# pdh930105/ARCQuant

Hardware: AMD Instinct MI355X
Metric: ARC-NVFP4 GEMM TFLOP/s (M=4096, N=KQ=4096, KE=64) (higher is better)
Workload: dtype f16

## Files before the change

arcquant_amd/agemm.py:

```python
from __future__ import annotations

import functools

import torch

from . import _lib
from ._lib import VARIANT_G16, VARIANT_G32, OUT_BF16, OUT_F32, ArcqError

_raw_stream = getattr(torch._C, "_cuda_getCurrentRawStream", None)


def _stream(t: torch.Tensor) -> int:
    if _raw_stream is not None:
        return _raw_stream(t.get_device())
    return torch.cuda.current_stream(t.device).cuda_stream


class _on:
    __slots__ = ("ctx",)

    def __init__(self, device):
        idx = device.index
        self.ctx = None if idx is None or idx == torch.cuda.current_device() else torch.cuda.device(device)

# ... 50 lines not shown

_OUT_CODES = {torch.bfloat16: OUT_BF16, torch.float32: OUT_F32}


def _out(out, M, N, out_dtype, like, who):
    code = _OUT_CODES.get(out_dtype)
    if code is None:
        raise RuntimeError(f"agemm.{who}: out_dtype must be bfloat16 or float32")
    if out is None:
        return torch.empty((M, N), dtype=out_dtype, device=like.device), code
    _need(out, out_dtype, "out", 2)
    if out.shape != (M, N):
        raise RuntimeError(f"agemm.{who}: out has the wrong shape, expected ({M}, {N})")
    return out, code


def _same_device(who: str, A: torch.Tensor, *ts):
    idx = A.get_device()
    if idx < 0:
        raise RuntimeError(f"agemm.{who}: the operands must live on the GPU (there is no CPU path)")
    for t in ts:
        if t is not None and t.get_device() != idx:
            raise RuntimeError(f"agemm.{who}: every operand must live on the GPU of the first one ({A.device}), got {t.device}")


@functools.lru_cache(maxsize=None)
def variant_for_kq(KQ: int) -> int:
    return int(_lib.lib().arcq_variant_for_kq(int(KQ)))


@functools.lru_cache(maxsize=None)
def sf_buffer_bytes(rows: int, K: int) -> int:
    return int(_lib.lib().arcq_sf_alloc_bytes(int(rows), int(K)))


@functools.lru_cache(maxsize=None)
def _sf_used(rows: int, K: int) -> int:
    return int(_lib.lib().arcq_sf_used_bytes(int(rows), int(K)))


@functools.lru_cache(maxsize=None)
def _repacked_bytes(N: int, K: int):
    L = _lib.lib()
    return int(L.arcq_repacked_w_bytes(N, K)), int(L.arcq_repacked_sf_bytes(N, K))


# ... 485 lines not shown
```

arcquant_amd/csrc/arcq_internal.hpp:

```cpp
#pragma once
#include <hip/hip_runtime.h>
#include <stdint.h>
#include <stdlib.h>

#include "../../include/arcq.h"

namespace arcq {

int fail(int code, const char* fmt, ...) __attribute__((format(printf, 2, 3)));

inline int env_int(const char* name, int dflt) {
  const char* e = getenv(name);
  return e ? atoi(e) : dflt;
}

constexpr int kMaxDevices = 64;
struct LdsOptIn {
  int granted[kMaxDevices];
};
int ensure_dynamic_lds(const void* kernel, LdsOptIn& cache, int bytes, const char* who);

struct LdsBytes {
  int launch, optin;
  LdsBytes(int bytes) : launch(bytes), optin(bytes) {}
// ... 99 lines not shown
  const uint8_t* RSF;
  void* D;
  uint32_t* out_slots;
  const int16_t* act_scatter;
  int M, N, KQ, KE, variant;
  float alpha_host;
  const float* alpha_dev;
  const uint16_t* bias;
  const uint16_t* residual;
  int out_dtype;
};
int gemm_fused_supported(int kind, int64_t M, int64_t N, int64_t KQ, int64_t KE);
int gemm_fused(const FusedArgs& f, hipStream_t stream);
int64_t gemm_skinny_workspace_bytes(int64_t M, int64_t N, int64_t K);
int64_t gemm_tile_workspace_bytes(int64_t M, int64_t N, int64_t K);
int64_t gemm_tile_silu_slots(int64_t M, int64_t N, int64_t K);
int64_t gemm_decode_silu_slots(int64_t M, int64_t N, int64_t K);
int gemm_splitk_finish(const GemmArgs& a, int splitk, hipStream_t stream);
int gemm_skinny(const GemmArgs& a, hipStream_t stream);
int64_t gemm_decode_workspace_bytes(int64_t M, int64_t N, int64_t K);
int gemm_decode(const GemmArgs& a, hipStream_t stream);
int gemm_tile(const GemmArgs& a, hipStream_t stream);
int gemm_tile_repacked(const GemmArgs& a, hipStream_t stream);
int gemm_regtile_cfg(int64_t M, int64_t N, int64_t K, int epilogue);
int gemm_regtile(const GemmArgs& a, int cfg, hipStream_t stream);
int gemm_regtile_fits(int64_t M, int64_t N, int64_t K, int b_layout);

struct KvWriteArgs {
  void* kv_data;
  void* kv_param;
  const int32_t *kv_indptr, *kv_indices, *last_page_offset;
  const void *k, *v, *k_param, *v_param;
  const int32_t* seqlen_indptr;
  int64_t ntok, B, L, layer, N, P;
  int format, dtype;
  bool quantize;
};
int kv_write(const KvWriteArgs& a, hipStream_t stream);
struct KvDecodeArgs {
  void* o;
  const void *q, *kv_data, *kv_param;
  const int32_t *kv_indptr, *kv_indices, *last_page_offset;
  int64_t B, Nq, L, layer, N, P, nnz;
  int format, dtype;
  void* workspace;
};
// ... 23 lines not shown
```

arcquant_amd/csrc/c_api.hip:

```cpp
#include <hip/hip_runtime.h>
#include <stdarg.h>
#include <stdio.h>
#include <string.h>

#include "arcq_device.hpp"
#include "arcq_internal.hpp"

namespace arcq {

static thread_local char g_err[512] = "";

int fail(int code, const char* fmt, ...) {
  va_list ap;
  va_start(ap, fmt);
  vsnprintf(g_err, sizeof(g_err), fmt, ap);
  va_end(ap);
  return code;
}

int ensure_dynamic_lds(const void* kernel, LdsOptIn& cache, int bytes, const char* who) {
  if (bytes <= 48 * 1024) return ARCQ_OK;
  int dev = 0;
  if (hipGetDevice(&dev) != hipSuccess) return fail(ARCQ_ERR_LAUNCH, "%s: hipGetDevice failed", who);
  const bool cached = dev >= 0 && dev < kMaxDevices;
// ... 95 lines not shown
                        int64_t M, int64_t KQ, int64_t KE, int variant, void* stream) {
  return quantize_x_dyn(X, reorder_index, QX, SFX, scale_out, state, M, KQ, KE, variant, (hipStream_t)stream);
}

int arcq_silu_mul_quantize_x_dyn(const void* GU, const int16_t* reorder_index, uint8_t* QX, uint8_t* SFX, float* scale_out, void* state,
                                 int64_t M, int64_t KQ, int64_t KE, int variant, int layout, void* stream) {
  return silu_mul_quantize_x_dyn(GU, reorder_index, QX, SFX, scale_out, state, M, KQ, KE, variant, layout, (hipStream_t)stream);
}

int arcq_absmax_scale(const void* X, int64_t n, float* scale_out, void* stream) {
  return absmax_scale(X, n, scale_out, (hipStream_t)stream);
}


static bool use_decode_v2(int64_t N) {
  static const int forced = env_int("ARCQ_DECODE", 0);
  if (forced == 1) return false;
  if (forced == 2) return true;
  return ((N + 127) / 128) * 4 >= 160;
}

int64_t arcq_gemm_workspace_bytes(int64_t M, int64_t N, int64_t K) {
  if (M <= 0 || N <= 0 || K <= 0) return 0;
  if (gemm_regtile_cfg(M, N, K, kEpiPlain)) return 0;
  if (M <= kSkinnyMaxM) return use_decode_v2(N) ? gemm_decode_workspace_bytes(M, N, K) : gemm_skinny_workspace_bytes(M, N, K);
  return gemm_tile_workspace_bytes(M, N, K);
}

int arcq_gemm_nvfp4(const uint8_t* A, const uint8_t* B, const uint8_t* SFA, const uint8_t* SFB, void* D, int64_t M, int64_t N,
                    int64_t K, float alpha_host, const float* alpha_dev, const void* bias, const void* residual, int out_dtype, void* workspace,
                    int64_t workspace_bytes, void* stream) {
  GemmRule r{"arcq_gemm_nvfp4"};
  const int rc = gemm_checks(r, A, B, SFA, SFB, D, nullptr, M, N, K, bias, residual, out_dtype);
  if (rc != ARCQ_OK) return rc < 0 ? rc : ARCQ_OK;
  const GemmArgs a = gemm_args(A, B, SFA, SFB, D, M, N, K, alpha_host, alpha_dev, bias, residual, out_dtype, workspace, workspace_bytes);
  if (const int cfg = gemm_regtile_cfg(M, N, K, kEpiPlain)) return gemm_regtile(a, cfg, (hipStream_t)stream);
  if (M <= kSkinnyMaxM) return use_decode_v2(N) ? gemm_decode(a, (hipStream_t)stream) : gemm_skinny(a, (hipStream_t)stream);
  return gemm_tile(a, (hipStream_t)stream);
}

int64_t arcq_gemm_silu_mul_slots(int64_t M, int64_t N, int64_t K) {
  if (M <= 0 || N <= 0 || K <= 0) return 0;
  return M <= kSkinnyMaxM ? gemm_decode_silu_slots(M, N, K) : gemm_tile_silu_slots(M, N, K);
}

int arcq_gemm_nvfp4_silu_mul(const uint8_t* A, const uint8_t* B, const uint8_t* SFA, const uint8_t* SFB, void* ACT, uint32_t* absmax_slots,
                             int64_t M, int64_t N, int64_t K, float alpha_host, const float* alpha_dev, const void* bias, void* stream) {
  GemmRule r{"arcq_gemm_nvfp4_silu_mul"};
  r.n_mult = 8; r.d = "ACT"; r.slots = true;
  const int rc = gemm_checks(r, A, B, SFA, SFB, ACT, absmax_slots, M, N, K, nullptr, nullptr, ARCQ_OUT_BF16);
  if (rc != ARCQ_OK) return rc < 0 ? rc : ARCQ_OK;
  GemmArgs a = gemm_args(A, B, SFA, SFB, ACT, M, N, K, alpha_host, alpha_dev, bias, nullptr, ARCQ_OUT_BF16, nullptr, 0);
  a.epilogue = kEpiSiluMul; a.absmax_slots = absmax_slots;
  if (bias && M <= kSkinnyMaxM) return fail(ARCQ_ERR_UNSUPPORTED, "%s: bias is supported by the tile kernel only (M > 16); decode uses arcq_linear_rmsnorm_silu_repacked", r.who);
  if (M <= kSkinnyMaxM) return gemm_decode(a, (hipStream_t)stream);
  return gemm_tile(a, (hipStream_t)stream);
}

// ... 25 lines not shown
int arcq_gemm_nvfp4_repacked_stream(const uint8_t* A, const uint8_t* RW, const uint8_t* SFA, const uint8_t* RSF, void* D, int64_t M, int64_t N,
                                    int64_t K, float alpha_host, const float* alpha_dev, const void* bias, const void* residual, int out_dtype,
                                    void* stream) {
  return gemm_repacked_entry(true, "arcq_gemm_nvfp4_repacked_stream", A, RW, SFA, RSF, D, M, N, K, alpha_host, alpha_dev, bias, residual, out_dtype, stream);
}

int arcq_gemm_nvfp4_repacked_silu_absmax(const uint8_t* A, const uint8_t* RW, const uint8_t* SFA, const uint8_t* RSF, void* D,
                                         uint32_t* absmax_slots, int64_t M, int64_t N, int64_t K, float alpha_host, const float* alpha_dev,
                                         void* stream) {
  GemmRule r{"arcq_gemm_nvfp4_repacked_silu_absmax"};
  r.n_mult = 4; r.max_m = 0; r.b = "RW"; r.sfb = "RSF"; r.slots = true;
  const int rc = gemm_checks(r, A, RW, SFA, RSF, D, absmax_slots, M, N, K, nullptr, nullptr, ARCQ_OUT_BF16);
  if (rc != ARCQ_OK) return rc < 0 ? rc : ARCQ_OK;
  GemmArgs a = gemm_args(A, nullptr, SFA, nullptr, D, M, N, K, alpha_host, alpha_dev, nullptr, nullptr, ARCQ_OUT_BF16, nullptr, 0);
  a.epilogue = kEpiSiluMul; a.absmax_slots = absmax_slots;
  return gemm_repacked(a, RW, RSF, (hipStream_t)stream);
}

static const int kRwDecodeCfg = 9;

static int rw_route(int64_t M, int64_t N, int64_t K, bool epi_aligned, int* cfg) {
  *cfg = 0;
  if (M <= 0 || N <= 0 || K <= 0 || (K % 64) || M > INT32_MAX / 2 || N > INT32_MAX / 2 || K > INT32_MAX / 2 || M * N > ((int64_t)1 << 40)) return 0;
  if (epi_aligned && gemm_repacked_supported(M, N, K)) return 1;
  *cfg = gemm_regtile_cfg(M, N, K, kEpiPlain);
  if (*cfg == 0 && M <= kSkinnyMaxM) *cfg = kRwDecodeCfg;
  if (*cfg) return gemm_regtile_fits(M, N, K, kBRepacked) ? 2 : 0;
  return 3;
}

int arcq_gemm_rw_route(int64_t M, int64_t N, int64_t K) {
  int cfg;
  return rw_route(M, N, K, true, &cfg);
}

int64_t arcq_gemm_rw_workspace_bytes(int64_t M, int64_t N, int64_t K) {
  int cfg;
  return rw_route(M, N, K, false, &cfg) == 3 ? gemm_tile_workspace_bytes(M, N, K) : 0;
}

int arcq_gemm_nvfp4_rw(const uint8_t* A, const uint8_t* RW, const uint8_t* SFA, const uint8_t* RSF, void* D, int64_t M, int64_t N, int64_t K,
                       float alpha_host, const float* alpha_dev, const void* bias, const void* residual, int out_dtype, void* workspace,
                       int64_t workspace_bytes, void* stream) {
  GemmRule r{"arcq_gemm_nvfp4_rw"};
  r.b = "RW"; r.sfb = "RSF";
  const int rc = gemm_checks(r, A, RW, SFA, RSF, D, nullptr, M, N, K, nullptr, nullptr, out_dtype);
// ... 108 lines not shown
```

arcquant_amd/csrc/gemm_tile.hip:

```cpp
#include <hip/hip_runtime.h>
#include <stdint.h>
#include <stdlib.h>

#include <type_traits>

#include "arcq_internal.hpp"
#include "gemm_common.hpp"
#include "gemm_tile_common.hpp"

namespace arcq {

#ifdef ARCQ_STREAM_STAMPS
static unsigned long long* g_tile_stamps = nullptr;
#ifndef ARCQ_TILE_REPACKED_UNIT
extern "C" void arcq_debug_set_tile_stamps(void* p) { g_tile_stamps = reinterpret_cast<unsigned long long*>(p); }
#endif
#define ARCQ_TILE_STAMP(k)                                                                                     \
  do {                                                                                                         \
    if (p.stamps && tid == 0) {                                                                                \
      unsigned long long t0_, t1_;                                                                             \
      asm volatile("s_memtime %0\n\ts_memrealtime %1\n\ts_waitcnt lgkmcnt(0)" : "=s"(t0_), "=s"(t1_)::"memory"); \
      p.stamps[(size_t)blockIdx.x * (2 * kTileStamps) + 2 * (k)] = t0_;                                        \
      p.stamps[(size_t)blockIdx.x * (2 * kTileStamps) + 2 * (k) + 1] = t1_;                                    \
    }                                                                                                          \
  } while (0)
#else
#define ARCQ_TILE_STAMP(k) do { } while (0)
#endif

#ifndef ARCQ_TILE_WIDE_STORES
#define ARCQ_TILE_WIDE_STORES 1
#endif

#ifndef ARCQ_TILE_BARRIER_AT_STEP_END
#define ARCQ_TILE_BARRIER_AT_STEP_END 0
#endif
#ifndef ARCQ_TILE_ROT
#define ARCQ_TILE_ROT 1
#endif

template <int BM, int BN, int WAVES_M, int WAVES_N, bool kMfma32, int kEpi, bool kStagger, bool kPipe, int kBLayout = kBRef>
__global__ __launch_bounds__(WAVES_M* WAVES_N * 64) void gemm_tile_kernel(TileParams p) {
  constexpr int kThreads = WAVES_M * WAVES_N * 64;
  constexpr int WM = BM / WAVES_M, WN = BN / WAVES_N;
  constexpr int kT = kMfma32 ? 32 : 16;
  constexpr int TM = WM / kT, TN = WN / kT;
  using acc_t = typename std::conditional<kMfma32, f32x16, f32x4>::type;
  constexpr int A_UNITS = (BM * 2 + kThreads - 1) / kThreads, B_UNITS = (BN * 2 + kThreads - 1) / kThreads;
  constexpr bool A_PARTIAL = (BM * 2) % kThreads != 0, B_PARTIAL = (BN * 2) % kThreads != 0;
  static_assert(!A_PARTIAL || A_UNITS == 1, "a partial A pass is a single pass");
  static_assert(!B_PARTIAL || B_UNITS == 1, "a partial B pass is a single pass");
  constexpr int A_TILE = BM * kRowBytes, B_TILE = BN * kRowBytes;

  extern __shared__ __attribute__((aligned(16))) unsigned char smem[];
  unsigned char* const lds_a0 = smem;
  unsigned char* const lds_b0 = smem + A_TILE;
  unsigned char* const lds_a1 = smem + A_TILE + B_TILE;
  unsigned char* const lds_b1 = smem + 2 * A_TILE + B_TILE;

  const int ntiles = p.tiles_m * p.tiles_n;
  int bid = blockIdx.x, split = 0;
  if (p.splits > 1) {
    split = bid / ntiles;
    bid -= split * ntiles;
  }
// ... 50 lines not shown
  }
  uint32_t b_q[B_UNITS], b_sf[B_UNITS];
  uint32_t b_live[B_UNITS];
  int b_slot[B_UNITS][4];
#pragma unroll
  for (int u = 0; u < B_UNITS; ++u) {
    const int unit = tid + u * kThreads, r = B_PARTIAL ? min(unit >> 1, BN - 1) : unit >> 1, h = unit & 1;
    const int row = n0 + r, rc = row < p.N ? row : p.N - 1;
    if constexpr (kBLayout == kBRepacked) {
      const uint32_t rb = (uint32_t)((rc >> 4) - (n0 >> 4));
      b_q[u] = rb * (uint32_t)rw_tiles * 1024u + h * 256 + (rc & 15) * 16;
      b_sf[u] = rb * (uint32_t)rw_tiles * 128u + h * 64 + (rc & 15) * 4;
    } else {
      b_q[u] = (uint32_t)(rc - n0) * (uint32_t)half_k + h * 16;
      b_sf[u] = (uint32_t)(sf_atom_offset(rc, 0, atoms_k) - sf_atom_offset(n0, 0, atoms_k)) + h * 2;
    }
    b_live[u] = row < p.N ? kSfLive : 0u;
#pragma unroll
    for (int j = 0; j < 4; ++j) b_slot[u][j] = kMfma32 ? lds_slot32(r, h * 4 + j) : lds_slot(r, h * 4 + j);
  }
  const int fa_base = kMfma32 ? lds_slot32(wr * WM + (lane & 31), lane >> 5) : lds_slot(wr * WM + (lane & 15), lane >> 4);
  const int fb_base = kMfma32 ? lds_slot32(wc * WN + (lane & 31), lane >> 5) : lds_slot(wc * WN + (lane & 15), lane >> 4);
  acc_t acc[TM][TN];
#pragma unroll
  for (int i = 0; i < TM; ++i)
#pragma unroll
    for (int j = 0; j < TN; ++j)
#pragma unroll
      for (int r = 0; r < (kMfma32 ? 16 : 4); ++r) acc[i][j][r] = 0.f;

  Staged sa[A_UNITS], sb[B_UNITS];
  auto load_step = [&](int atom) {
    atom = __builtin_amdgcn_readfirstlane(atom);
    const StageStep sa_step = stage_step(atom), sb_step = kBLayout == kBRepacked ? stage_step_rw(atom) : sa_step;
#pragma unroll
    for (int u = 0; u < A_UNITS; ++u) sa[u] = stage_load(a_src, a_q[u], a_sf[u], sa_step);
#pragma unroll
    for (int u = 0; u < B_UNITS; ++u) sb[u] = stage_load(b_src, b_q[u], b_sf[u], sb_step);
  };
  auto store_step = [&](unsigned char* la, unsigned char* lb) {
#pragma unroll
    for (int u = 0; u < A_UNITS; ++u)
      if (!A_PARTIAL || tid < BM * 2) stage_store(la, a_slot[u], sa[u], a_live[u]);
#pragma unroll
    for (int u = 0; u < B_UNITS; ++u)
      if (!B_PARTIAL || tid < BN * 2) stage_store(lb, b_slot[u], sb[u], b_live[u]);
  };
  auto mma_step = [&](const unsigned char* la, const unsigned char* lb) {
    if constexpr (kMfma32) {
#pragma unroll
      for (int ks = 0; ks < 4; ++ks) {
        Frag8 fa[TM], fb[TN];
// ... 199 lines not shown
#pragma unroll
        for (int j = 0; j < TN; ++j)
          if constexpr (!kMfma32)
            acc[2 * pr + ii][j] = __builtin_amdgcn_mfma_f32_16x16x32_f16(fb[ks][j].v, fq[q][ii].v, acc[2 * pr + ii][j], 0, 0, 0);
      pieces(q);
#pragma unroll
      for (int m8 = 0; m8 < (TM == 8 ? 2 * TN : 0); ++m8) {
        __builtin_amdgcn_sched_group_barrier(0x008, 1, 0);
        __builtin_amdgcn_sched_group_barrier(0x002, 2, 0);
      }
      __builtin_amdgcn_sched_barrier(0);
    }
    __syncthreads();
  };

  load_step(a_begin);
  Staged sa0[A_UNITS], sb0[B_UNITS];
#pragma unroll
  for (int u = 0; u < A_UNITS; ++u) sa0[u] = sa[u];
#pragma unroll
  for (int u = 0; u < B_UNITS; ++u) sb0[u] = sb[u];
  load_step(min(a_begin + 1, a_end - 1));
  __builtin_amdgcn_sched_barrier(0);
#pragma unroll
  for (int u = 0; u < A_UNITS; ++u)
    if (!A_PARTIAL || tid < BM * 2) stage_store(lds_a0, a_slot[u], sa0[u], a_live[u]);
#pragma unroll
  for (int u = 0; u < B_UNITS; ++u)
    if (!B_PARTIAL || tid < BN * 2) stage_store(lds_b0, b_slot[u], sb0[u], b_live[u]);
  if (kStagger && late) {
    store_step(lds_a1, lds_b1);
    load_step(min(a_begin + 2, a_end - 1));
  }
  __syncthreads();
  if constexpr (kRotate) {
#pragma unroll
    for (int j = 0; j < TN; ++j) head_b[j] = rd_frag(lds_b0, fb_base, 0, j);
    head_a[0] = rd_frag(lds_a0, fa_base, 0, 0);
    head_a[1] = rd_frag(lds_a0, fa_base, 0, 1);
  }
  int kt = a_begin;
#ifndef ARCQ_EXPERIMENT_GENERAL_EPILOGUE
  float alpha_dev = 1.0f;
  if (p.alpha_dev) alpha_dev = *reinterpret_cast<const __attribute__((address_space(4))) float*>(reinterpret_cast<uintptr_t>(p.alpha_dev));
  asm volatile("" : "+s"(alpha_dev));
#endif
  if (WAVES_M * WAVES_N == 8 && wave >= 4) __builtin_amdgcn_s_setprio(1);
  ARCQ_TILE_STAMP(1);
  if constexpr (kPipe) {
    for (; kt + 1 < a_end; kt += 2) {
      k_step_pipe(kt, lds_a0, lds_b0, lds_a1, lds_b1);
      k_step_pipe(kt + 1, lds_a1, lds_b1, lds_a0, lds_b0);
    }
    if (kt < a_end) k_step_pipe(kt, lds_a0, lds_b0, lds_a1, lds_b1);
  } else {
    for (; kt + 1 < a_end; kt += 2) {
      k_step(kt, lds_a0, lds_b0, lds_a1, lds_b1);
      k_step(kt + 1, lds_a1, lds_b1, lds_a0, lds_b0);
    }
    if (kt < a_end) k_step(kt, lds_a0, lds_b0, lds_a1, lds_b1);
  }
  ARCQ_TILE_STAMP(2);

#ifdef ARCQ_EXPERIMENT_GENERAL_EPILOGUE
  const float alpha = p.alpha_host * (p.alpha_dev ? *p.alpha_dev : 1.0f);
#else
  const float alpha = p.alpha_host * alpha_dev;
#endif
  const bool vec_ok = (p.N & 3) == 0;
  uint32_t act_max = 0;
  [[maybe_unused]] auto interior_epilogue = [&](auto has_bias, auto has_res) __attribute__((always_inline)) {
    constexpr bool kBias = decltype(has_bias)::value, kRes = decltype(has_res)::value;
    constexpr bool kSilu = kEpi == kEpiSiluMul;
    constexpr uint32_t kElem = kSilu ? 1 : 2;
    unsigned char* const tile_d = reinterpret_cast<unsigned char*>(p.D) + ((size_t)m0 * p.N + n0) * kElem;
    const unsigned char* const tile_r = kRes ? reinterpret_cast<const unsigned char*>(p.residual) + ((size_t)m0 * p.N + n0) * 2 : nullptr;
    uint32_t t = tid;
    asm volatile("" : "+v"(t));
    const uint32_t lane_row = (t >> 6) / WAVES_N * WM + (t & 15), lane_col = (t >> 6) % WAVES_N * WN + 4 * ((t >> 4) & 3);
    uint32_t off = lane_row * (uint32_t)p.N + lane_col;
    const uint32_t row_step = 16u * (uint32_t)p.N;
    constexpr bool kWide = ARCQ_TILE_WIDE_STORES && !kSilu && TN % 2 == 0;
    typedef uint32_t u32x4_a8 __attribute__((ext_vector_type(4), aligned(8)));
    [[maybe_unused]] const uint32_t g4 = (t >> 4) & 3;
    [[maybe_unused]] uint32_t off_w = off - 4 * g4 + ((g4 & 1) ? 16 + 4 * (g4 - 1) : 4 * g4);
    [[maybe_unused]] uint2 held = make_uint2(0, 0);
    float bias_f[TN][4];
    if constexpr (kBias) {
#pragma unroll
      for (int j = 0; j < TN; ++j) {
        const uint2 b = *reinterpret_cast<const uint2*>(p.bias + n0 + lane_col + j * 16);
        bias_f[j][0] = bf16_bits_to_f32(b.x & 0xffffu); bias_f[j][1] = bf16_bits_to_f32(b.x >> 16);
        bias_f[j][2] = bf16_bits_to_f32(b.y & 0xffffu); bias_f[j][3] = bf16_bits_to_f32(b.y >> 16);
      }
    }
    uint2 res_cur[TN], res_nxt[TN];
    auto res_load = [&](uint32_t o, uint2 (&r)[TN]) {
#pragma unroll
      for (int j = 0; j < TN; ++j) r[j] = *reinterpret_cast<const uint2*>(tile_r + (size_t)o * 2 + j * 32);
    };
    if constexpr (kRes) res_load(off, res_cur);
#pragma unroll
    for (int i = 0; i < TM; ++i) {
      if constexpr (kRes) { if (i + 1 < TM) res_load(off + row_step, res_nxt); }
#pragma unroll
      for (int j = 0; j < TN; ++j) {
        float d[4] = {alpha * acc[i][j][0], alpha * acc[i][j][1], alpha * acc[i][j][2], alpha * acc[i][j][3]};
        if constexpr (kSilu) {
          if constexpr (kBias) {
#pragma unroll
            for (int r = 0; r < 4; r += 2) {
              round2_to_bf16(d[r], d[r + 1]);
              d[r] += bias_f[j][r];
              d[r + 1] += bias_f[j][r + 1];
            }
          }
          const uint32_t y01 = pack_bf16x2_hw(d[0], d[1]), y23 = pack_bf16x2_hw(d[2], d[3]);
          const uint32_t a0 = silu_mul_bf16(y01 & 0xffffu, y01 >> 16), a1 = silu_mul_bf16(y23 & 0xffffu, y23 >> 16);
          *reinterpret_cast<uint32_t*>(tile_d + (size_t)off + j * 16) = a0 | (a1 << 16);
          act_max = max(act_max, max(a0 & 0x7fffu, a1 & 0x7fffu));
        } else {
          if constexpr (kBias) {
#pragma unroll
            for (int r = 0; r < 4; r += 2) {
              round2_to_bf16(d[r], d[r + 1]);
              d[r] += bias_f[j][r];
              d[r + 1] += bias_f[j][r + 1];
            }
          }
// ... 2 lines not shown
#pragma unroll
            for (int r = 0; r < 4; r += 2) {
              round2_to_bf16(d[r], d[r + 1]);
              d[r] += bf16_bits_to_f32(rw[r >> 1] & 0xffffu);
              d[r + 1] += bf16_bits_to_f32(rw[r >> 1] >> 16);
            }
          }
          const uint2 pk = make_uint2(pack_bf16x2_hw(d[0], d[1]), pack_bf16x2_hw(d[2], d[3]));
          if constexpr (kWide) {
            if (j & 1) {
              const auto lo = __builtin_amdgcn_permlane16_swap(held.x, pk.x, false, false);
              const auto hi = __builtin_amdgcn_permlane16_swap(held.y, pk.y, false, false);
              const u32x4_a8 v = {lo[0], hi[0], lo[1], hi[1]};
              *reinterpret_cast<u32x4_a8*>(tile_d + (size_t)off_w * 2 + (j >> 1) * 64) = v;
            } else {
              held = pk;
            }
          } else {
            *reinterpret_cast<uint2*>(tile_d + (size_t)off * 2 + j * 32) = pk;
          }
        }
        if (i == 0 && j == 0) ARCQ_TILE_STAMP(3);
      }
      if constexpr (kRes) {
#pragma unroll
        for (int j = 0; j < TN; ++j) res_cur[j] = res_nxt[j];
      }
      off += row_step;
      off_w += row_step;
    }
  };
  auto store4 = [&](int m, int n, float d0, float d1, float d2, float d3, bool pre, uint2 bias2, uint2 res2) __attribute__((always_inline)) {
    if (m >= p.M || n >= p.N) return;
    const uint32_t bw[2] = {bias2.x, bias2.y}, rw[2] = {res2.x, res2.y};
    auto bias_at = [&](int r) { return bf16_bits_to_f32(pre ? (bw[r >> 1] >> (16 * (r & 1))) & 0xffffu : (uint32_t)p.bias[n + r]); };
    if (kEpi == kEpiSiluMul) {
      uint32_t y[4] = {f32_to_bf16_bits(alpha * d0), f32_to_bf16_bits(alpha * d1), f32_to_bf16_bits(alpha * d2), f32_to_bf16_bits(alpha * d3)};
      if (p.bias) {
#pragma unroll
        for (int e = 0; e < 4; ++e) y[e] = f32_to_bf16_bits(bf16_bits_to_f32(y[e]) + bias_at(e));
      }
      const uint32_t a0 = silu_mul_bf16(y[0], y[1]);
      const uint32_t a1 = silu_mul_bf16(y[2], y[3]);
      *reinterpret_cast<uint32_t*>(reinterpret_cast<uint16_t*>(p.D) + (size_t)m * (p.N >> 1) + (n >> 1)) = a0 | (a1 << 16);
      act_max = max(act_max, max(a0 & 0x7fffu, a1 & 0x7fffu));
      return;
    }
    if (p.splits > 1) {
      *reinterpret_cast<float4*>(p.partial + ((size_t)split * p.M + m) * p.N + n) = make_float4(d0, d1, d2, d3);
      return;
    }
    float d[4] = {alpha * d0, alpha * d1, alpha * d2, alpha * d3};
// ... 5 lines not shown
    if (p.residual) {
#pragma unroll
      for (int r = 0; r < 4; ++r)
        if (pre || n + r < p.N) {
          const float res = bf16_bits_to_f32(pre ? (rw[r >> 1] >> (16 * (r & 1))) & 0xffffu : (uint32_t)p.residual[(size_t)m * p.N + n + r]);
          d[r] = (p.out_dtype == ARCQ_OUT_F32 ? d[r] : bf16_bits_to_f32(f32_to_bf16_bits(d[r]))) + res;
        }
    }
    if (p.out_dtype == ARCQ_OUT_F32) {
      float* o = reinterpret_cast<float*>(p.D) + (size_t)m * p.N + n;
      if (vec_ok) *reinterpret_cast<float4*>(o) = make_float4(d[0], d[1], d[2], d[3]);
      else for (int r = 0; r < 4; ++r) if (n + r < p.N) o[r] = d[r];
    } else {
      uint16_t* o = reinterpret_cast<uint16_t*>(p.D) + (size_t)m * p.N + n;
      if (vec_ok) *reinterpret_cast<uint2*>(o) = make_uint2(pack_bf16x2(d[0], d[1]), pack_bf16x2(d[2], d[3]));
      else for (int r = 0; r < 4; ++r) if (n + r < p.N) o[r] = (uint16_t)f32_to_bf16_bits(d[r]);
    }
  };
#ifdef ARCQ_EXPERIMENT_GENERAL_EPILOGUE
  constexpr bool kInteriorPath = false;
#else
  constexpr bool kInteriorPath = !kMfma32;
#endif
  bool interior = false;
  if constexpr (kInteriorPath)
    interior = m0 + BM <= p.M && n0 + BN <= p.N && vec_ok && p.splits <= 1 && p.out_dtype == ARCQ_OUT_BF16 && (int64_t)BM * p.N < (1ll << 31) &&
               ((reinterpret_cast<uintptr_t>(p.bias) | reinterpret_cast<uintptr_t>(p.residual)) & 7) == 0;
  if (interior) {
    if constexpr (kInteriorPath) {
      using T = std::true_type;
      using F = std::false_type;
      if constexpr (kEpi == kEpiSiluMul) {
        if (p.bias) interior_epilogue(T{}, F{});
        else interior_epilogue(F{}, F{});
      } else if (p.bias) {
        if (p.residual) interior_epilogue(T{}, T{});
        else interior_epilogue(T{}, F{});
      } else {
        if (p.residual) interior_epilogue(F{}, T{});
        else interior_epilogue(F{}, F{});
      }
    }
  } else if constexpr (kMfma32) {
#pragma unroll
    for (int i = 0; i < TM; ++i)
#pragma unroll
      for (int j = 0; j < TN; ++j) {
        const int m = m0 + wr * WM + i * 32 + (lane & 31);
#pragma unroll
        for (int g = 0; g < 4; ++g) {
          const int n = n0 + wc * WN + j * 32 + 8 * g + 4 * (lane >> 5);
// ... 35 lines not shown
#pragma unroll
        for (int j = 0; j < TN; ++j) {
          store4(mb + i * 16, nb + j * 16, acc[i][j][0], acc[i][j][1], acc[i][j][2], acc[i][j][3], false, make_uint2(0, 0), make_uint2(0, 0));
          if (i == 0 && j == 0) ARCQ_TILE_STAMP(3);
        }
    }
  }
  ARCQ_TILE_STAMP(4);
  if (kEpi == kEpiSiluMul) {
    __shared__ uint32_t wave_max[WAVES_M * WAVES_N];
#pragma unroll
    for (int sh = 32; sh > 0; sh >>= 1) act_max = max(act_max, (uint32_t)__shfl_down((int)act_max, sh, 64));
    if (lane == 0) wave_max[wave] = act_max;
    __syncthreads();
    if (tid == 0) {
      uint32_t m = 0;
#pragma unroll
      for (int w = 0; w < WAVES_M * WAVES_N; ++w) m = max(m, wave_max[w]);
      p.slots[blockIdx.x] = m;
    }
  }
}

struct TileCfg { int id, bm, bn, waves; };
static constexpr TileCfg kTileCfgs[] = {{1, 128, 128, 4}, {2, 256, 256, 4}, {3, 256, 256, 8}, {4, 128, 256, 4}, {5, 256, 256, 8}, {6, 128, 128, 4},
                                        {7, 64, 256, 4}, {8, 32, 256, 4}, {9, 128, 128, 4}, {10, 128, 256, 8}, {11, 256, 128, 8}, {12, 128, 128, 8},
                                        {13, 64, 256, 8}, {14, 64, 128, 8}, {15, 64, 64, 4}, {16, 64, 128, 4}, {17, 128, 64, 4}};
static const TileCfg& tile_cfg(int id) {
  for (const TileCfg& c : kTileCfgs)
    if (c.id == id) return c;
  return kTileCfgs[2];
}

static int tile_cfg_override() {
  static const int v = env_int("ARCQ_TILE_CFG", 0);
  return v;
}
static int tile_split_override() {
  static const int v = env_int("ARCQ_TILE_SPLIT", 0);
  return v;
}
static bool tile_stagger() {
  static const int v = env_int("ARCQ_TILE_STAGGER", 0);
  return v != 0;
}
static bool tile_pipe() {
// ... 25 lines not shown
  p.splits = 1; p.atoms_per_split = a.K / 64; p.partial = nullptr;
  p.epi = a.epilogue; p.slots = a.absmax_slots;
#ifdef ARCQ_STREAM_STAMPS
  p.stamps = g_tile_stamps;
#endif
  if (allow_split && a.epilogue == kEpiPlain) {
    tile_split(a.M, a.N, a.K, BM, BN, &p.splits, &p.atoms_per_split);
    if (p.splits > 1) {
      const int64_t need = (int64_t)p.splits * a.M * a.N * (int64_t)sizeof(float);
      if (!a.workspace || a.workspace_bytes < need)
        return fail(ARCQ_ERR_WORKSPACE, "arcq_gemm_nvfp4: split-K needs %lld B of workspace, got %lld", (long long)need,
                    (long long)a.workspace_bytes);
      p.partial = reinterpret_cast<float*>(a.workspace);
    }
  }
  if (((int64_t)a.K + 255) / 256 * 256 * 128 > 0xffffffffll)
    return fail(ARCQ_ERR_SHAPE, "arcq_gemm_nvfp4 (tile): K = %lld: a tile's rows of an operand exceed 32-bit offsets", (long long)a.K);
  const int lds = 2 * (BM + BN) * kRowBytes;
  const dim3 grid((unsigned)(p.tiles_m * p.tiles_n * p.splits)), block(WAVES_M * WAVES_N * 64);
  const char* who = "arcq_gemm_nvfp4 (tile)";
  constexpr bool kCanStagger = WAVES_M * WAVES_N == 8 && BM == 256 && BN == 256;
  const bool pipe = tile_pipe(), stagger = !pipe && kCanStagger && tile_stagger();
  int rc;
  if (!pipe && !stagger) rc = launch_kernel<gemm_tile_kernel<BM, BN, WAVES_M, WAVES_N, kMfma32, kEpi, false, false, kBLayout>>(grid, block, lds, stream, who, p);
  else if (pipe) rc = launch_kernel<gemm_tile_kernel<BM, BN, WAVES_M, WAVES_N, kMfma32, kEpi, false, true, kBLayout>>(grid, block, lds, stream, who, p);
  else rc = launch_kernel<gemm_tile_kernel<BM, BN, WAVES_M, WAVES_N, kMfma32, kEpi, kCanStagger, false, kBLayout>>(grid, block, lds, stream, who, p);
  if (rc != ARCQ_OK) return rc;
  if (p.splits > 1) return gemm_splitk_finish(a, p.splits, stream);
  return ARCQ_OK;
}

static int tile_choice(int64_t M, int64_t N, int64_t K) {
  const int64_t t256 = ((M + 255) / 256) * ((N + 255) / 256);
  if (t256 >= 192) return 3;
  if (M <= 32) return 8;
  if (M <= 64) return 7;
  const int64_t t10 = ((M + 127) / 128) * ((N + 255) / 256);
  if (t10 <= 64 || t10 == 128 || (t10 > 224 && t10 <= 256) || (K >= 8192 && t10 >= 96 && t10 <= 256)) return 10;
  return 1;
}

static int effective_cfg(int64_t M, int64_t N, int64_t K, bool* may_split) {
  int id = tile_cfg_override();
  if (id == 0) id = tile_choice(M, N, K);
  id = tile_cfg(id).id;
  *may_split = !(id >= 2 && id <= 6) && id != 9;
  return id;
}

#ifndef ARCQ_TILE_REPACKED_UNIT
int64_t gemm_tile_silu_slots(int64_t M, int64_t N, int64_t K) {
  bool sp;
  const TileCfg& c = tile_cfg(effective_cfg(M, N, K, &sp));
  return ((M + c.bm - 1) / c.bm) * ((N + c.bn - 1) / c.bn);
}

int64_t gemm_tile_workspace_bytes(int64_t M, int64_t N, int64_t K) {
  int s = 1, per = 0;
  bool sp;
  const TileCfg& c = tile_cfg(effective_cfg(M, N, K, &sp));
  if (sp) tile_split(M, N, K, c.bm, c.bn, &s, &per);
  return s > 1 ? (int64_t)s * M * N * (int64_t)sizeof(float) : 0;
}
#endif

template <int kEpi, int kBLayout>
static int gemm_tile_epi(const GemmArgs& a, hipStream_t stream) {
// ... 8 lines not shown
    case 8: return launch_tile<32, 256, 1, 4, false, kEpi, kBLayout>(a, stream, sp);
    case 10: return launch_tile<128, 256, 2, 4, false, kEpi, kBLayout>(a, stream, sp);
    case 11: return launch_tile<256, 128, 4, 2, false, kEpi, kBLayout>(a, stream, sp);
    case 12: return launch_tile<128, 128, 2, 4, false, kEpi, kBLayout>(a, stream, sp);
    case 13: return launch_tile<64, 256, 1, 8, false, kEpi, kBLayout>(a, stream, sp);
    case 14: return launch_tile<64, 128, 2, 4, false, kEpi, kBLayout>(a, stream, sp);
    case 15: return launch_tile<64, 64, 2, 2, false, kEpi, kBLayout>(a, stream, sp);
    case 16: return launch_tile<64, 128, 2, 2, false, kEpi, kBLayout>(a, stream, sp);
    case 17: return launch_tile<128, 64, 2, 2, false, kEpi, kBLayout>(a, stream, sp);
    default: return launch_tile<256, 256, 2, 4, false, kEpi, kBLayout>(a, stream);
  }
}

#ifndef ARCQ_TILE_REPACKED_UNIT
int gemm_tile(const GemmArgs& a, hipStream_t stream) {
  if (a.b_layout == kBRepacked) return gemm_tile_repacked(a, stream);
  return a.epilogue == kEpiSiluMul ? gemm_tile_epi<kEpiSiluMul, kBRef>(a, stream) : gemm_tile_epi<kEpiPlain, kBRef>(a, stream);
}
#else
int gemm_tile_repacked(const GemmArgs& a, hipStream_t stream) {
  return a.epilogue == kEpiSiluMul ? gemm_tile_epi<kEpiSiluMul, kBRepacked>(a, stream) : gemm_tile_epi<kEpiPlain, kBRepacked>(a, stream);
}
#endif

}
```

arcquant_amd/csrc/gemm_tile_common.hpp:

```cpp
#pragma once
#include <hip/hip_runtime.h>
#include <stdint.h>

#include "arcq_internal.hpp"
#include "gemm_common.hpp"

namespace arcq {

struct TileParams {
  const uint8_t* A;
  const uint8_t* B;
  const uint8_t* SFA;
  const uint8_t* SFB;
  void* D;
  const float* alpha_dev;
  const uint16_t* bias;
  const uint16_t* residual;
  int M, N, K;
  float alpha_host;
  int out_dtype;
  int tiles_m, tiles_n;
  int splits, atoms_per_split;
  float* partial;
  int epi;
  unsigned int* slots;
#ifdef ARCQ_STREAM_STAMPS
  unsigned long long* stamps;
#endif
};
constexpr int kTileStamps = 5;

constexpr int kBK = 64;
constexpr int kRowBytes = kBK * 2;

__device__ __forceinline__ int lds_slot(int r, int ks) { return r * kRowBytes + ((ks ^ (r & 7)) << 4); }
__device__ __forceinline__ int lds_slot32(int r, int ks) { return r * kRowBytes + ((ks ^ ((r >> 1) & 7)) << 4); }

struct Staged {
  uint4 q;
  uint32_t sf;
};

typedef uint32_t u32x4 __attribute__((ext_vector_type(4)));
typedef __amdgpu_buffer_rsrc_t buf_rsrc;

__device__ __forceinline__ buf_rsrc stage_rsrc(const uint8_t* base, uint32_t bytes) {
  return __builtin_amdgcn_make_buffer_rsrc(const_cast<uint8_t*>(base), 0, (int)bytes, 0x00020000);
}

struct StageSrc {
  buf_rsrc q, sf;
};
struct StageStep {
// ... 51 lines not shown
```

Baseline: 1440.

## Overlap tile GEMM epilogue with final K-step MFMAs in dedicated kernel

Adds a separate compilation unit with an overlapped-tail variant of the 256x256, 8-wave pipelined tile kernel. It peels the last K step and interleaves each row's epilogue (alpha scale, bias and residual loads, bf16 stores) with the MFMAs of the remaining rows, using sched_group_barrier to alternate matrix and vector work. The aim is to hide epilogue latency behind tensor math instead of running it after the main loop. It also adds a debug mode that forces routing to this tile kernel instead of regtile, plus specialised launches per bias/residual combination; the cost is more register pressure and more kernel variants.

```diff
diff --git a/arcquant_amd/agemm.py b/arcquant_amd/agemm.py
--- a/arcquant_amd/agemm.py
+++ b/arcquant_amd/agemm.py
@@ -96,6 +96,13 @@
     for t in ts:
         if t is not None and t.get_device() != idx:
             raise RuntimeError(f"agemm.{who}: every operand must live on the GPU of the first one ({A.device}), got {t.device}")
+
+
+def _debug_set_tile_overlap_tail(mode: int) -> None:
+    fn = _lib.lib().arcq_debug_set_tile_overlap_tail
+    fn.restype, fn.argtypes = None, [_lib._i32]
+    fn(int(mode))
+    rw_route.cache_clear()
 
 
 @functools.lru_cache(maxsize=None)
diff --git a/arcquant_amd/csrc/arcq_internal.hpp b/arcquant_amd/csrc/arcq_internal.hpp
--- a/arcquant_amd/csrc/arcq_internal.hpp
+++ b/arcquant_amd/csrc/arcq_internal.hpp
@@ -145,6 +145,8 @@
 int gemm_decode(const GemmArgs& a, hipStream_t stream);
 int gemm_tile(const GemmArgs& a, hipStream_t stream);
 int gemm_tile_repacked(const GemmArgs& a, hipStream_t stream);
+int tile_overlap_tail_mode();
+inline bool tile_overlap_tail_forced(int64_t M, int64_t N) { return tile_overlap_tail_mode() == 2 && M % 256 == 0 && N % 256 == 0; }
 int gemm_regtile_cfg(int64_t M, int64_t N, int64_t K, int epilogue);
 int gemm_regtile(const GemmArgs& a, int cfg, hipStream_t stream);
 int gemm_regtile_fits(int64_t M, int64_t N, int64_t K, int b_layout);
diff --git a/arcquant_amd/csrc/c_api.hip b/arcquant_amd/csrc/c_api.hip
--- a/arcquant_amd/csrc/c_api.hip
+++ b/arcquant_amd/csrc/c_api.hip
@@ -141,6 +141,7 @@
 
 int64_t arcq_gemm_workspace_bytes(int64_t M, int64_t N, int64_t K) {
   if (M <= 0 || N <= 0 || K <= 0) return 0;
+  if (tile_overlap_tail_forced(M, N)) return gemm_tile_workspace_bytes(M, N, K);
   if (gemm_regtile_cfg(M, N, K, kEpiPlain)) return 0;
   if (M <= kSkinnyMaxM) return use_decode_v2(N) ? gemm_decode_workspace_bytes(M, N, K) : gemm_skinny_workspace_bytes(M, N, K);
   return gemm_tile_workspace_bytes(M, N, K);
@@ -153,6 +154,7 @@
   const int rc = gemm_checks(r, A, B, SFA, SFB, D, nullptr, M, N, K, bias, residual, out_dtype);
   if (rc != ARCQ_OK) return rc < 0 ? rc : ARCQ_OK;
   const GemmArgs a = gemm_args(A, B, SFA, SFB, D, M, N, K, alpha_host, alpha_dev, bias, residual, out_dtype, workspace, workspace_bytes);
+  if (tile_overlap_tail_forced(M, N)) return gemm_tile(a, (hipStream_t)stream);
   if (const int cfg = gemm_regtile_cfg(M, N, K, kEpiPlain)) return gemm_regtile(a, cfg, (hipStream_t)stream);
   if (M <= kSkinnyMaxM) return use_decode_v2(N) ? gemm_decode(a, (hipStream_t)stream) : gemm_skinny(a, (hipStream_t)stream);
   return gemm_tile(a, (hipStream_t)stream);
@@ -224,6 +226,7 @@
 static int rw_route(int64_t M, int64_t N, int64_t K, bool epi_aligned, int* cfg) {
   *cfg = 0;
   if (M <= 0 || N <= 0 || K <= 0 || (K % 64) || M > INT32_MAX / 2 || N > INT32_MAX / 2 || K > INT32_MAX / 2 || M * N > ((int64_t)1 << 40)) return 0;
+  if (tile_overlap_tail_forced(M, N)) return 3;
   if (epi_aligned && gemm_repacked_supported(M, N, K)) return 1;
   *cfg = gemm_regtile_cfg(M, N, K, kEpiPlain);
   if (*cfg == 0 && M <= kSkinnyMaxM) *cfg = kRwDecodeCfg;
diff --git a/arcquant_amd/csrc/gemm_tile.hip b/arcquant_amd/csrc/gemm_tile.hip
--- a/arcquant_amd/csrc/gemm_tile.hip
+++ b/arcquant_amd/csrc/gemm_tile.hip
@@ -11,9 +11,11 @@
 namespace arcq {
 
 #ifdef ARCQ_STREAM_STAMPS
+#ifndef ARCQ_TILE_OT_UNIT
 static unsigned long long* g_tile_stamps = nullptr;
 #ifndef ARCQ_TILE_REPACKED_UNIT
 extern "C" void arcq_debug_set_tile_stamps(void* p) { g_tile_stamps = reinterpret_cast<unsigned long long*>(p); }
+#endif
 #endif
 #define ARCQ_TILE_STAMP(k)                                                                                     \
   do {                                                                                                         \
@@ -39,8 +41,17 @@
 #define ARCQ_TILE_ROT 1
 #endif
 
+#ifndef ARCQ_TILE_OT_UNIT
 template <int BM, int BN, int WAVES_M, int WAVES_N, bool kMfma32, int kEpi, bool kStagger, bool kPipe, int kBLayout = kBRef>
 __global__ __launch_bounds__(WAVES_M* WAVES_N * 64) void gemm_tile_kernel(TileParams p) {
+  constexpr bool kOverlapTail = false;
+  [[maybe_unused]] constexpr int kEpiOps = 0;
+#else
+template <int BM, int BN, int WAVES_M, int WAVES_N, int kEpi, int kBLayout, int kEpiOps>
+__global__ __launch_bounds__(WAVES_M* WAVES_N * 64) void gemm_tile_ot_kernel(TileParams p) {
+  static_assert(kEpiOps >= 0 && kEpiOps < (kEpi == kEpiSiluMul ? 2 : 4), "bit 0 bias, bit 1 residual (SiLU * up has no residual)");
+  constexpr bool kMfma32 = false, kStagger = false, kPipe = true, kOverlapTail = true;
+#endif
   constexpr int kThreads = WAVES_M * WAVES_N * 64;
   constexpr int WM = BM / WAVES_M, WN = BN / WAVES_N;
   constexpr int kT = kMfma32 ? 32 : 16;
@@ -137,12 +148,14 @@
   const int fa_base = kMfma32 ? lds_slot32(wr * WM + (lane & 31), lane >> 5) : lds_slot(wr * WM + (lane & 15), lane >> 4);
   const int fb_base = kMfma32 ? lds_slot32(wc * WN + (lane & 31), lane >> 5) : lds_slot(wc * WN + (lane & 15), lane >> 4);
   acc_t acc[TM][TN];
-#pragma unroll
-  for (int i = 0; i < TM; ++i)
-#pragma unroll
-    for (int j = 0; j < TN; ++j)
-#pragma unroll
-      for (int r = 0; r < (kMfma32 ? 16 : 4); ++r) acc[i][j][r] = 0.f;
+  if constexpr (!kOverlapTail) {
+#pragma unroll
+    for (int i = 0; i < TM; ++i)
+#pragma unroll
+      for (int j = 0; j < TN; ++j)
+#pragma unroll
+        for (int r = 0; r < (kMfma32 ? 16 : 4); ++r) acc[i][j][r] = 0.f;
+  }
 
   Staged sa[A_UNITS], sb[B_UNITS];
   auto load_step = [&](int atom) {
@@ -388,6 +401,16 @@
   for (int u = 0; u < B_UNITS; ++u) sb0[u] = sb[u];
   load_step(min(a_begin + 1, a_end - 1));
   __builtin_amdgcn_sched_barrier(0);
+  if constexpr (kOverlapTail) {
+#pragma unroll
+    for (int i = 0; i < TM; ++i)
+#pragma unroll
+      for (int j = 0; j < TN; ++j) {
+        acc[i][j] = acc_t{};
+        asm volatile("" : "+v"(acc[i][j]));
+      }
+    __builtin_amdgcn_sched_barrier(0);
+  }
 #pragma unroll
   for (int u = 0; u < A_UNITS; ++u)
     if (!A_PARTIAL || tid < BM * 2) stage_store(lds_a0, a_slot[u], sa0[u], a_live[u]);
@@ -413,7 +436,18 @@
 #endif
   if (WAVES_M * WAVES_N == 8 && wave >= 4) __builtin_amdgcn_s_setprio(1);
   ARCQ_TILE_STAMP(1);
-  if constexpr (kPipe) {
+  [[maybe_unused]] int tail_buf = 0;
+  if constexpr (kOverlapTail) {
+    static_assert(kRotate, "the final step is entered with head fragments");
+    for (; kt + 2 < a_end; kt += 2) {
+      k_step_pipe(kt, lds_a0, lds_b0, lds_a1, lds_b1);
+      k_step_pipe(kt + 1, lds_a1, lds_b1, lds_a0, lds_b0);
+    }
+    if (kt + 1 < a_end) {
+      k_step_pipe(kt, lds_a0, lds_b0, lds_a1, lds_b1);
+      tail_buf = A_TILE + B_TILE;
+    }
+  } else if constexpr (kPipe) {
     for (; kt + 1 < a_end; kt += 2) {
       k_step_pipe(kt, lds_a0, lds_b0, lds_a1, lds_b1);
       k_step_pipe(kt + 1, lds_a1, lds_b1, lds_a0, lds_b0);
@@ -426,7 +460,7 @@
     }
     if (kt < a_end) k_step(kt, lds_a0, lds_b0, lds_a1, lds_b1);
   }
-  ARCQ_TILE_STAMP(2);
+  if constexpr (!kOverlapTail) ARCQ_TILE_STAMP(2);
 
 #ifdef ARCQ_EXPERIMENT_GENERAL_EPILOGUE
   const float alpha = p.alpha_host * (p.alpha_dev ? *p.alpha_dev : 1.0f);
@@ -451,13 +485,19 @@
     [[maybe_unused]] const uint32_t g4 = (t >> 4) & 3;
     [[maybe_unused]] uint32_t off_w = off - 4 * g4 + ((g4 & 1) ? 16 + 4 * (g4 - 1) : 4 * g4);
     [[maybe_unused]] uint2 held = make_uint2(0, 0);
+    constexpr bool kPackedBias = kOverlapTail && kBias && kRes;
     float bias_f[TN][4];
+    [[maybe_unused]] uint2 bias_v[TN];
     if constexpr (kBias) {
 #pragma unroll
       for (int j = 0; j < TN; ++j) {
         const uint2 b = *reinterpret_cast<const uint2*>(p.bias + n0 + lane_col + j * 16);
-        bias_f[j][0] = bf16_bits_to_f32(b.x & 0xffffu); bias_f[j][1] = bf16_bits_to_f32(b.x >> 16);
-        bias_f[j][2] = bf16_bits_to_f32(b.y & 0xffffu); bias_f[j][3] = bf16_bits_to_f32(b.y >> 16);
+        if constexpr (kPackedBias) {
+          bias_v[j] = b;
+        } else {
+          bias_f[j][0] = bf16_bits_to_f32(b.x & 0xffffu); bias_f[j][1] = bf16_bits_to_f32(b.x >> 16);
+          bias_f[j][2] = bf16_bits_to_f32(b.y & 0xffffu); bias_f[j][3] = bf16_bits_to_f32(b.y >> 16);
+        }
       }
     }
     uint2 res_cur[TN], res_nxt[TN];
@@ -466,11 +506,14 @@
       for (int j = 0; j < TN; ++j) r[j] = *reinterpret_cast<const uint2*>(tile_r + (size_t)o * 2 + j * 32);
     };
     if constexpr (kRes) res_load(off, res_cur);
-#pragma unroll
-    for (int i = 0; i < TM; ++i) {
-      if constexpr (kRes) { if (i + 1 < TM) res_load(off + row_step, res_nxt); }
-#pragma unroll
-      for (int j = 0; j < TN; ++j) {
+    auto row_quad = [&](int i, int j) __attribute__((always_inline)) {
+      {
+        if constexpr (kPackedBias) {
+          uint2 b = bias_v[j];
+          asm volatile("" : "+v"(b.x), "+v"(b.y));
+          bias_f[j][0] = bf16_bits_to_f32(b.x & 0xffffu); bias_f[j][1] = bf16_bits_to_f32(b.x >> 16);
+          bias_f[j][2] = bf16_bits_to_f32(b.y & 0xffffu); bias_f[j][3] = bf16_bits_to_f32(b.y >> 16);
+        }
         float d[4] = {alpha * acc[i][j][0], alpha * acc[i][j][1], alpha * acc[i][j][2], alpha * acc[i][j][3]};
         if constexpr (kSilu) {
           if constexpr (kBias) {
@@ -519,12 +562,75 @@
         }
         if (i == 0 && j == 0) ARCQ_TILE_STAMP(3);
       }
-      if constexpr (kRes) {
-#pragma unroll
-        for (int j = 0; j < TN; ++j) res_cur[j] = res_nxt[j];
-      }
-      off += row_step;
-      off_w += row_step;
+    };
+    if constexpr (!kOverlapTail) {
+#pragma unroll
+      for (int i = 0; i < TM; ++i) {
+        if constexpr (kRes) { if (i + 1 < TM) res_load(off + row_step, res_nxt); }
+#pragma unroll
+        for (int j = 0; j < TN; ++j) row_quad(i, j);
+        if constexpr (kRes) {
+#pragma unroll
+          for (int j = 0; j < TN; ++j) res_cur[j] = res_nxt[j];
+        }
+        off += row_step;
+        off_w += row_step;
+      }
+    } else {
+      auto row_open = [&](int i) __attribute__((always_inline)) {
+        if constexpr (kRes) { if (i + 1 < TM) res_load(off + row_step, res_nxt); }
+      };
+      auto row_close = [&]() __attribute__((always_inline)) {
+        if constexpr (kRes) {
+#pragma unroll
+          for (int j = 0; j < TN; ++j) res_cur[j] = res_nxt[j];
+        }
+        off += row_step;
+        off_w += row_step;
+      };
+      constexpr int kQ = TM;
+      constexpr bool kUnder = !kSilu;
+      constexpr int kValu = 3 + (kBias ? 5 : 0) + (kRes ? 7 : 0);
+      const unsigned char* const fla = lds_a0 + tail_buf;
+      const unsigned char* const flb = lds_b0 + tail_buf;
+      Frag8 fb1[TN], fq[kQ][2];
+      fq[0][0] = head_a[0];
+      fq[0][1] = head_a[1];
+#pragma unroll
+      for (int j = 0; j < TN; ++j) fb1[j] = rd_frag(flb, fb_base, 1, j);
+#pragma unroll
+      for (int b = 0; b < kQ; ++b) {
+        if (b + 1 < kQ) {
+          fq[b + 1][0] = rd_frag(fla, fa_base, (b + 1) & 1, 2 * ((b + 1) >> 1));
+          fq[b + 1][1] = rd_frag(fla, fa_base, (b + 1) & 1, 2 * ((b + 1) >> 1) + 1);
+        }
+        if (kUnder && b >= 2) row_open(b - 2);
+        __builtin_amdgcn_sched_barrier(0);
+#pragma unroll
+        for (int s = 0; s < TN; ++s) {
+#pragma unroll
+          for (int m8 = 2 * s; m8 < 2 * s + 2; ++m8)
+            if constexpr (!kMfma32)
+              acc[2 * (b >> 1) + m8 / TN][m8 % TN] = __builtin_amdgcn_mfma_f32_16x16x32_f16(((b & 1) ? fb1[m8 % TN] : head_b[m8 % TN]).v, fq[b][m8 / TN].v,
+                                                                                             acc[2 * (b >> 1) + m8 / TN][m8 % TN], 0, 0, 0);
+          if (kUnder && b >= 2) {
+            row_quad(b - 2, s);
+            __builtin_amdgcn_sched_group_barrier(0x008, 1, 0);
+            __builtin_amdgcn_sched_group_barrier(0x002, kValu, 0);
+            __builtin_amdgcn_sched_group_barrier(0x008, 1, 0);
+          }
+          __builtin_amdgcn_sched_barrier(0);
+        }
+        if (kUnder && b >= 2) row_close();
+      }
+      ARCQ_TILE_STAMP(2);
+#pragma unroll
+      for (int i = kUnder ? TM - 2 : 0; i < TM; ++i) {
+        row_open(i);
+#pragma unroll
+        for (int j = 0; j < TN; ++j) row_quad(i, j);
+        row_close();
+      }
     }
   };
   auto store4 = [&](int m, int n, float d0, float d1, float d2, float d3, bool pre, uint2 bias2, uint2 res2) __attribute__((always_inline)) {
@@ -576,11 +682,14 @@
 #else
   constexpr bool kInteriorPath = !kMfma32;
 #endif
+  static_assert(!kOverlapTail || kInteriorPath, "the final step carries the interior epilogue");
   bool interior = false;
-  if constexpr (kInteriorPath)
+  if constexpr (kInteriorPath && !kOverlapTail)
     interior = m0 + BM <= p.M && n0 + BN <= p.N && vec_ok && p.splits <= 1 && p.out_dtype == ARCQ_OUT_BF16 && (int64_t)BM * p.N < (1ll << 31) &&
                ((reinterpret_cast<uintptr_t>(p.bias) | reinterpret_cast<uintptr_t>(p.residual)) & 7) == 0;
-  if (interior) {
+  if constexpr (kOverlapTail) {
+    interior_epilogue(std::bool_constant<(kEpiOps & 1) != 0>{}, std::bool_constant<(kEpiOps & 2) != 0>{});
+  } else if (interior) {
     if constexpr (kInteriorPath) {
       using T = std::true_type;
       using F = std::false_type;
@@ -662,6 +771,36 @@
   }
 }
 
+#ifdef ARCQ_TILE_OT_UNIT
+static int g_tile_overlap_tail = 1;
+int tile_overlap_tail_mode() { return g_tile_overlap_tail; }
+extern "C" void arcq_debug_set_tile_overlap_tail(int mode) { g_tile_overlap_tail = mode < 0 ? 0 : mode > 2 ? 2 : mode; }
+
+template <int kEpi, int kBLayout, int kEpiOps>
+static int launch_ot(const TileParams& p, dim3 grid, hipStream_t stream) {
+  return launch_kernel<gemm_tile_ot_kernel<256, 256, 2, 4, kEpi, kBLayout, kEpiOps>>(grid, dim3(512), 2 * (256 + 256) * kRowBytes, stream,
+                                                                                   "arcq_gemm_nvfp4 (tile, overlapped tail)", p);
+}
+template <int kEpi, int kBLayout>
+static int launch_ot_ops(const TileParams& p, dim3 grid, hipStream_t stream) {
+  const int ops = (p.bias ? 1 : 0) | (p.residual ? 2 : 0);
+  if constexpr (kEpi == kEpiSiluMul) {
+    return ops & 1 ? launch_ot<kEpi, kBLayout, 1>(p, grid, stream) : launch_ot<kEpi, kBLayout, 0>(p, grid, stream);
+  } else {
+    switch (ops) {
+      case 1: return launch_ot<kEpi, kBLayout, 1>(p, grid, stream);
+      case 2: return launch_ot<kEpi, kBLayout, 2>(p, grid, stream);
+      case 3: return launch_ot<kEpi, kBLayout, 3>(p, grid, stream);
+      default: return launch_ot<kEpi, kBLayout, 0>(p, grid, stream);
+    }
+  }
+}
+int launch_tile_overlap_tail(const TileParams& p, int epi, int b_layout, dim3 grid, hipStream_t stream) {
+  if (epi == kEpiSiluMul) return b_layout == kBRepacked ? launch_ot_ops<kEpiSiluMul, kBRepacked>(p, grid, stream) : launch_ot_ops<kEpiSiluMul, kBRef>(p, grid, stream);
+  return b_layout == kBRepacked ? launch_ot_ops<kEpiPlain, kBRepacked>(p, grid, stream) : launch_ot_ops<kEpiPlain, kBRef>(p, grid, stream);
+}
+#else
+
 struct TileCfg { int id, bm, bn, waves; };
 static constexpr TileCfg kTileCfgs[] = {{1, 128, 128, 4}, {2, 256, 256, 4}, {3, 256, 256, 8}, {4, 128, 256, 4}, {5, 256, 256, 8}, {6, 128, 128, 4},
                                         {7, 64, 256, 4}, {8, 32, 256, 4}, {9, 128, 128, 4}, {10, 128, 256, 8}, {11, 256, 128, 8}, {12, 128, 128, 8},
@@ -733,7 +872,12 @@
   constexpr bool kCanStagger = WAVES_M * WAVES_N == 8 && BM == 256 && BN == 256;
   const bool pipe = tile_pipe(), stagger = !pipe && kCanStagger && tile_stagger();
   int rc;
-  if (!pipe && !stagger) rc = launch_kernel<gemm_tile_kernel<BM, BN, WAVES_M, WAVES_N, kMfma32, kEpi, false, false, kBLayout>>(grid, block, lds, stream, who, p);
+  bool overlap_tail = false;
+  if constexpr (BM == 256 && BN == 256 && WAVES_M * WAVES_N == 8 && !kMfma32 && !ARCQ_TILE_BARRIER_AT_STEP_END)
+    overlap_tail = pipe && (kEpi == kEpiSiluMul ? tile_overlap_tail_mode() == 2 : tile_overlap_tail_mode() != 0) && a.M % BM == 0 && a.N % BN == 0 && p.splits <= 1 && a.out_dtype == ARCQ_OUT_BF16 &&
+                   (int64_t)BM * a.N < (1ll << 31) && ((reinterpret_cast<uintptr_t>(a.bias) | reinterpret_cast<uintptr_t>(a.residual)) & 7) == 0;
+  if (overlap_tail) rc = launch_tile_overlap_tail(p, kEpi, kBLayout, grid, stream);
+  else if (!pipe && !stagger) rc = launch_kernel<gemm_tile_kernel<BM, BN, WAVES_M, WAVES_N, kMfma32, kEpi, false, false, kBLayout>>(grid, block, lds, stream, who, p);
   else if (pipe) rc = launch_kernel<gemm_tile_kernel<BM, BN, WAVES_M, WAVES_N, kMfma32, kEpi, false, true, kBLayout>>(grid, block, lds, stream, who, p);
   else rc = launch_kernel<gemm_tile_kernel<BM, BN, WAVES_M, WAVES_N, kMfma32, kEpi, kCanStagger, false, kBLayout>>(grid, block, lds, stream, who, p);
   if (rc != ARCQ_OK) return rc;
@@ -753,7 +897,7 @@
 
 static int effective_cfg(int64_t M, int64_t N, int64_t K, bool* may_split) {
   int id = tile_cfg_override();
-  if (id == 0) id = tile_choice(M, N, K);
+  if (id == 0) id = tile_overlap_tail_forced(M, N) ? 3 : tile_choice(M, N, K);
   id = tile_cfg(id).id;
   *may_split = !(id >= 2 && id <= 6) && id != 9;
   return id;
@@ -808,5 +952,6 @@
   return a.epilogue == kEpiSiluMul ? gemm_tile_epi<kEpiSiluMul, kBRepacked>(a, stream) : gemm_tile_epi<kEpiPlain, kBRepacked>(a, stream);
 }
 #endif
-
-}
+#endif
+
+}
diff --git a/arcquant_amd/csrc/gemm_tile_common.hpp b/arcquant_amd/csrc/gemm_tile_common.hpp
--- a/arcquant_amd/csrc/gemm_tile_common.hpp
+++ b/arcquant_amd/csrc/gemm_tile_common.hpp
@@ -29,6 +29,7 @@
 #endif
 };
 constexpr int kTileStamps = 5;
+int launch_tile_overlap_tail(const TileParams& p, int epi, int b_layout, dim3 grid, hipStream_t stream);
 
 constexpr int kBK = 64;
 constexpr int kRowBytes = kBK * 2;
diff --git a/arcquant_amd/csrc/gemm_tile_ot.hip b/arcquant_amd/csrc/gemm_tile_ot.hip
--- /dev/null
+++ b/arcquant_amd/csrc/gemm_tile_ot.hip
@@ -0,0 +1,2 @@
+#define ARCQ_TILE_OT_UNIT
+#include "gemm_tile.hip"
```

Result: faster. 1459 (median of 6 runs) (+1.3%).
